# Keyteer/Mixed-precision_LU_Factorization

Hardware: AMD Instinct MI355X
Metric: LU GFLOP/s at N=32768 (1/2/4/8 GPUs); IR iterations to ||r||/||b||<1e-12 (higher is better)
Workload: dtype f64

## Files before the change

### mixed-precision_lu_factorization_amd/csrc/laswp.hip

```cpp
#include "mpf_internal.h"

constexpr int LASWP_CPB = 16;

__global__ __launch_bounds__(256) void laswp_plan_kernel(const int *ipiv, int k, int cols, MovedList *out) {
    __shared__ int slot[HP_MAXCOLS];
    __shared__ int rowof[2 * HP_MAXCOLS];
    __shared__ int content[2 * HP_MAXCOLS];
    __shared__ int used[2 * HP_MAXCOLS];
    __shared__ int count;
    const int t = threadIdx.x;
    for (int s = t; s < 2 * cols; s += 256) { content[s] = s; used[s] = s < cols; rowof[s] = s < cols ? k + s : -1; }
    if (t == 0) count = 0;
    __syncthreads();
    if (t < cols) {
        const int p = ipiv[t] - 1;
        int s;
        if (p < k + cols) s = p - k;
        else {
            int first = t;
            for (int i = 0; i < t; ++i)
                if (ipiv[i] - 1 == p) { first = i; break; }
            s = cols + first;
            if (first == t) { rowof[s] = p; used[s] = 1; }
        }
// ... 308 lines not shown
int launch_cvt_f64_f32(mpf_ctx *c, const double *A, int64_t lda, float *W, int64_t ldw, int64_t rows, int64_t cols) {
    if (rows <= 0 || cols <= 0) return 0;
    if ((cols + 63) / 64 > 65535) { c->err = "cvt: too many columns"; return -1; }
    dim3 grid((unsigned)((rows + 63) / 64), (unsigned)((cols + 63) / 64));
    cvt_a64_wt32_kernel<<<grid, 256, 0, c->stream>>>(A, lda, W, ldw, rows, cols);
    MPF_HIP_TRY(c, hipGetLastError());
    return 0;
}
int launch_cvt_f32_f64(mpf_ctx *c, const float *W, int64_t ldw, double *A, int64_t lda, int64_t rows, int64_t cols) {
    if (rows <= 0 || cols <= 0) return 0;
    if ((cols + 63) / 64 > 65535) { c->err = "cvt: too many columns"; return -1; }
    dim3 grid((unsigned)((rows + 63) / 64), (unsigned)((cols + 63) / 64));
    cvt_wt32_a64_kernel<<<grid, 256, 0, c->stream>>>(W, ldw, A, lda, rows, cols);
    MPF_HIP_TRY(c, hipGetLastError());
    return 0;
}

__global__ void lazy_init_map_kernel(int *F, int *G, long long n) {
    const long long i = (long long)blockIdx.x * 256 + threadIdx.x;
    if (i < n) { F[i] = (int)i; G[i] = (int)i; }
}
__global__ __launch_bounds__(512) void lazy_update_map_kernel(int *F, int *G, const MovedList *ml) {
    int n = ml->n;
    if (n > LASWP_MAXMOVED) n = LASWP_MAXMOVED;
    const int t = threadIdx.x;
    int v = 0;
    if (t < n) v = F[ml->dst[t]];
    __syncthreads();
    if (t < n) { const int s = ml->src[t]; F[s] = v; G[v] = s; }
}
__global__ __launch_bounds__(256) void lazy_gather_kernel(const double *__restrict__ A, long long lda, long long n, long long r0,
                                                         int w, const int *__restrict__ G, double *__restrict__ T, long long ldt) {
    const long long d = r0 + (long long)blockIdx.x * 256 + threadIdx.x;
    if (d >= n) return;
    const long long sr = G[d];
    const int c0 = blockIdx.y * 16;
#pragma unroll 8
    for (int c = c0; c < c0 + 16 && c < w; ++c) T[(d - r0) + (long long)c * ldt] = A[sr + (long long)c * lda];
}
__global__ __launch_bounds__(256) void lazy_scatter_kernel(const double *__restrict__ A, long long lda, long long n, long long r0,
                                                          int w, const int *__restrict__ F, double *__restrict__ T, long long ldt) {
    const long long r = r0 + (long long)blockIdx.x * 256 + threadIdx.x;
    if (r >= n) return;
    const long long d = (long long)F[r] - r0;
    const int c0 = blockIdx.y * 16;
#pragma unroll 4
    for (int c = c0; c < c0 + 16 && c < w; ++c) T[d + (long long)c * ldt] = A[r + (long long)c * lda];
}
__global__ __launch_bounds__(256) void lazy_copyback_kernel(double *__restrict__ A, long long lda, long long n, long long r0, int w,
                                                           const double *__restrict__ T, long long ldt) {
    const long long r = r0 + (long long)blockIdx.x * 256 + threadIdx.x;
    if (r >= n) return;
    const int c0 = blockIdx.y * 16;
#pragma unroll 4
    for (int c = c0; c < c0 + 16 && c < w; ++c) A[r + (long long)c * lda] = T[(r - r0) + (long long)c * ldt];
}

int launch_lazy_left_swaps(mpf_ctx *c, double *A, int64_t lda, int64_t N, int nb, int npanels, const MovedList *lists, int sb,
                           int world, int rank) {
    if (npanels < 2) return 0;
    if (sb < 1 || world > 1) sb = 1;
    const int gather = c->tune.lazy_gather;
    int *Gmap = c->Fmap + N;
    lazy_init_map_kernel<<<(int)((N + 255) / 256), 256, 0, c->stream>>>(c->Fmap, Gmap, N);
    for (int p = npanels - 1; p >= 1; --p) {
        lazy_update_map_kernel<<<1, 512, 0, c->stream>>>(c->Fmap, Gmap, lists + p);
        if (p % sb) continue;
        const int64_t r0 = (int64_t)p * nb;
        const int64_t rows = N - r0;
        if (rows <= 0) continue;
        for (int b = p - sb; b < p; ++b) {
            if (world > 1 && b % world != rank) continue;
            const int w = nb;
            dim3 grid((unsigned)((rows + 255) / 256), (unsigned)((w + 15) / 16));
            double *Ab = A + (int64_t)(world > 1 ? b / world : b) * nb * lda;
            if (gather) lazy_gather_kernel<<<grid, 256, 0, c->stream>>>(Ab, lda, N, r0, w, Gmap, c->perm_tmp, rows);
            else lazy_scatter_kernel<<<grid, 256, 0, c->stream>>>(Ab, lda, N, r0, w, c->Fmap, c->perm_tmp, rows);
            lazy_copyback_kernel<<<grid, 256, 0, c->stream>>>(Ab, lda, N, r0, w, c->perm_tmp, rows);
        }
    }
    MPF_HIP_TRY(c, hipGetLastError());
    return 0;
}
```

### mixed-precision_lu_factorization_amd/csrc/mpf_host.cpp

```cpp
#include "mpf_internal.h"
#include "../../include/MPF.h"
#include <climits>
#include <cstdio>
#include <cstdlib>
#include <cstring>
#include <cmath>
#include <iostream>
#include <vector>
#include <mutex>
#include <functional>
#include <chrono>

static thread_local std::string g_noctx_err;

namespace {
struct OptDesc { const char *name, *env; size_t off; bool wide; long long lo, hi; };
#define OPT_I(field, env, lo, hi) {#field, env, offsetof(MpfTuning, field), false, lo, hi}
#define OPT_L(field, env, lo, hi) {#field, env, offsetof(MpfTuning, field), true, lo, hi}
const OptDesc kOpts[] = {
    OPT_I(safe_pivots, "MPF_SAFE_PIVOTS", 0, 1),
    OPT_I(chain_pipeline, "MPF_CHAIN_PIPELINE", 0, 1),
    OPT_L(chain_pipeline_below, "MPF_CHAIN_PIPELINE_BELOW", 0, 1ll << 40),
    OPT_I(fp16_work32, "MPF_FP16_WORK32", 0, 1),
    OPT_I(superpanel_fp16, "MPF_SUPERPANEL", 0, 8),
    OPT_I(superpanel_fp64, "MPF_SUPERPANEL_FP64", 1, 8),
    OPT_I(no_lookahead, "MPF_NO_LOOKAHEAD", 0, 1),
    OPT_I(verbose, "MPF_VERBOSE", 0, 1),
    OPT_I(timeline, "MPF_TIMELINE", 0, 1),
    OPT_L(hp_spin_limit, "MPF_HP_SPIN_LIMIT", 1, 1ll << 31),
    OPT_L(hp_gate_ticks, "MPF_HP_GATE_TICKS", 0, 1ll << 40),
    OPT_I(hp_acq_fence, "MPF_HP_ACQ_FENCE", 0, 1),
    OPT_I(hp_window, "MPF_HP_WINDOW", -1, 1 << 30),
    OPT_I(hgemm_pad, "MPF_HGEMM_PAD", 0, 65536),
    OPT_I(hgemm_split_pad, "MPF_HGEMM_SPLIT_PAD", 0, 65536),
    OPT_I(hgemm_big, "MPF_HGEMM_BIG", 0, 1),
    OPT_I(hgemm_big_tile, "MPF_HGEMM_BIG_TILE", 0, 5),
    OPT_I(hgemm_mfma16, "MPF_HGEMM_MFMA16", 0, 1),
    OPT_I(dgemm_dma, "MPF_DGEMM_DMA", 0, 1),
    OPT_I(lazy_gather, "MPF_LAZY_GATHER", 0, 1),
    OPT_I(dpanel_fused_form, "MPF_DPANEL_FUSED", 0, 1),
    OPT_I(dist_instalments, "MPF_DIST_INSTALMENTS", 0, 1),
    OPT_L(dist_instalment_min_bytes, "MPF_DIST_INSTALMENT_MIN_BYTES", 0, 1ll << 40),
    OPT_I(generic_fused, "MPF_GENERIC_FUSED", 0, 1),
    OPT_I(fp64_rowmajor, "MPF_FP64_ROWMAJOR", 0, 1),
    OPT_L(fp64_rowmajor_min_n, "MPF_FP64_ROWMAJOR_MIN_N", 0, 1ll << 40),
    OPT_I(trsm_laswp_fused, "MPF_TRSM_LASWP_FUSED", 0, 1),
    OPT_I(fp64_two_lanes, "MPF_FP64_TWO_LANES", 0, 1 << 30),
    OPT_I(fp64_lane_a_pct, "MPF_FP64_LANE_A_PCT", 20, 90),
    OPT_I(event_timers, "MPF_EVENT_TIMERS", 0, 2),
    OPT_I(dist_world1_loop, "MPF_DIST_WORLD1_LOOP", 0, 1),
    OPT_I(gesv_fp64_tflops, "MPF_GESV_FP64_TFLOPS", 0, 1000),
    OPT_I(gate_wait_value, "MPF_GATE_WAIT_VALUE", 0, 1),
    OPT_I(host_sink, "MPF_HOST_SINK", 0, 1),
    OPT_I(sink_trace, "MPF_SINK_TRACE", 0, 1),
    OPT_I(hp_half_slabs, "MPF_HP_HALF_SLABS", 0, 1),
    OPT_I(hp_half_slabs_rows, "MPF_HP_HALF_SLABS_ROWS", 256, 32768),
    OPT_I(hp_local_xcd, "MPF_HP_LOCAL_XCD", 0, 2),
    OPT_I(host_late_parts, "MPF_HOST_LATE_PARTS", 0, 4),
    OPT_L(host_late_min_n, "MPF_HOST_LATE_MIN_N", 0, 1ll << 40),
    OPT_I(host_first_pct, "MPF_HOST_FIRST_PCT", 5, 100),
    OPT_I(host_late_q_pct, "MPF_HOST_LATE_Q_PCT", 1, 1000),
    OPT_L(host_sink_min_n, "MPF_HOST_SINK_MIN_N", 0, 1ll << 40),
    OPT_I(dist_solve_p2p, "MPF_DIST_SOLVE_P2P", 0, 1),
#ifdef MPF_PROBE
    OPT_I(hp_stamp, "MPF_HP_STAMP", 0, 1),
    OPT_I(hp_r256_upto, "MPF_HP_R256_UPTO", 0, 1 << 30),
    OPT_I(dgemm_w8, "MPF_DGEMM_W8", 0, 1),
    OPT_I(gemm_lds_pad, "MPF_GEMM_LDS_PAD", 0, 65536),
    OPT_I(hgemm_big_reg, "MPF_HGEMM_BIG_REG", 0, 1),
    OPT_I(hgemm_dbg, "MPF_HGEMM_DBG", 0, 8191),
#endif
};
#undef OPT_I
#undef OPT_L
void opt_store(MpfTuning &t, const OptDesc &d, long long v) {
    if (v < d.lo) v = d.lo;
    if (v > d.hi) v = d.hi;
    char *p = (char *)&t + d.off;
    if (d.wide) *(long long *)p = v; else *(int *)p = (int)v;
}
long long opt_load(const MpfTuning &t, const OptDesc &d) {
    const char *p = (const char *)&t + d.off;
    return d.wide ? *(const long long *)p : (long long)*(const int *)p;
}
void tuning_from_env(MpfTuning &t) {
    for (const OptDesc &d : kOpts)
        if (const char *e = getenv(d.env)) if (*e) opt_store(t, d, atoll(e));
}
}

static int fail(mpf_ctx *c, int code, const std::string &msg) {
    if (c) c->err = msg; else g_noctx_err = msg;
    return code;
}

extern "C" {

int mpf_create(mpf_ctx **out, int device) {
    if (!out) return -1;
    *out = nullptr;
    int ndev = 0;
    hipError_t e = hipGetDeviceCount(&ndev);
    if (e != hipSuccess || ndev == 0) return fail(nullptr, -3, "No HIP devices available.");
    if (device < 0 || device >= ndev) return fail(nullptr, -1, "mpf_create: bad device index");
    mpf_ctx *c = new mpf_ctx();
    tuning_from_env(c->tune);
    c->device = device;
    if (hipSetDevice(device) != hipSuccess) { delete c; return fail(nullptr, -2, "hipSetDevice failed"); }
    hipDeviceProp_t prop;
    if (hipGetDeviceProperties(&prop, device) == hipSuccess) c->num_cus = prop.multiProcessorCount;
    if (hipStreamCreateWithFlags(&c->stream, hipStreamNonBlocking) != hipSuccess) { delete c; return fail(nullptr, -2, "hipStreamCreate failed"); }
    c->own_stream = true;
    {
        int lo = 0, hi = 0;
        hipDeviceGetStreamPriorityRange(&lo, &hi);
        if (hipStreamCreateWithPriority(&c->pstream, hipStreamNonBlocking, hi) != hipSuccess) c->pstream = nullptr;
        if (hipStreamCreateWithPriority(&c->tstream, hipStreamNonBlocking, hi) != hipSuccess) c->tstream = nullptr;
    }
    if (hipMalloc((void **)&c->ws, sizeof(MpfWorkspace)) != hipSuccess) { hipStreamDestroy(c->stream); delete c; return fail(nullptr, -2, "hipMalloc(workspace) failed"); }
    hipMemset(c->ws, 0, sizeof(MpfWorkspace));
    if (hipExtMallocWithFlags((void **)&c->hp_signal, 8, hipMallocSignalMemory) != hipSuccess) { c->hp_signal = nullptr; (void)hipGetLastError(); }
    else hipMemset(c->hp_signal, 0, 8);
// ... 437 lines not shown
        const int64_t ns = has_next ? pc2 : n;
        rc = ev.timed(st.ms_trsm, S, [&] { return launch_dtrsm_llnu(c, pc, ns, Ap, lda, A12, lda); });
        if (rc) break;
        rc = ev.timed(st.ms_gemm, S, [&] {
            int e = o.trailing != MPF_TRAIL_FP64 ? launch_cvt_l21(c, Ap + pc, lda, n, pc, o.trailing == MPF_TRAIL_FP16X3) : 0;
            if (!e) e = trail_gemm(c, o, n, ns, pc, Ap + pc, A12, A12 + pc, lda);
            return e; });
        if (rc) break;
        count_gemm(st, o, n, ns, pc);
        if (!has_next) break;
        hipEvent_t e1 = ev.get(), e2 = ev.get();
        hipEventRecord(e1, S);
        hipEvent_t e2p = nullptr, e2t = nullptr;
        int rcp = 0;
        const bool piped = chain_pipelined(c, ev, st, o, d_A, lda, N, nx, pc2, d_ipiv, c->lists + (nx / nb), e1, &e2p, &e2t, &rcp) == 0;
        if (piped) rc = rcp;
        else {
            hipStreamWaitEvent(P, e1, 0);
            StreamSwap sw(c, P);
            double *Anx = d_A + nx * lda + nx;
            MovedList *ml = c->lists + (nx / nb);
            rc = ev.timed(st.ms_hpanel, P, [&] {
                return launch_hgetf2(c, Anx, lda, nullptr, 0, (int)(N - nx), pc2, (int)nx, d_ipiv + nx, nullptr, 0, ml, 0, o.trailing == MPF_TRAIL_FP64 ? HP_FP64_WINDOW_ROWS : 0); });
            if (!rc) rc = ev.timed(st.ms_dpanel, P, [&] {
                int e = launch_laswp_from_list(c, d_A + nx * lda, lda, pc2, ml);
                if (!e) e = launch_dgetf2_npv(c, Anx, lda, (int)(N - nx), pc2, o.fused_panel, (int)nx);
                return e;
            });
        }
        if (rc) break;
        if (!piped) hipEventRecord(e2, P);
        st.panels++;
        if (n > pc2) {
            rc = ev.timed(st.ms_laswp, S, [&] {
                return launch_laswp_from_list(c, d_A + (nx + pc2) * lda, lda, N - nx - pc2, c->lists + (k / nb)); });
            if (rc) break;
            double *A12r = A12 + (int64_t)pc2 * lda;
            rc = ev.timed(st.ms_trsm, S, [&] { return launch_dtrsm_llnu(c, pc, n - pc2, Ap, lda, A12r, lda); });
            if (rc) break;
            if (sink) sink_notify(c, (int)(k / nb) + 1, S);
            rc = ev.timed(st.ms_gemm, S, [&] { return trail_gemm(c, o, n, n - pc2, pc, Ap + pc, A12r, A12r + pc, lda); });
            if (rc) break;
            count_gemm(st, o, n, n - pc2, pc);
        }
        if (piped) { hipStreamWaitEvent(S, e2p, 0); hipStreamWaitEvent(S, e2t, 0); }
        else hipStreamWaitEvent(S, e2, 0);
        rc = ev.timed(st.ms_laswp, S, [&] {
            const int64_t s0 = nx + pc2;
            const int64_t sw = (N - s0) < nb ? (N - s0) : nb;
            return sw > 0 ? launch_laswp_from_list(c, d_A + s0 * lda, lda, sw, c->lists + (nx / nb)) : 0;
        });
        if (o.verbose) printf("panel k=%lld rows=%lld cols=%d (look-ahead)\n", (long long)nx, (long long)(N - nx), pc2);
    }
    if (sink) {
        hipEvent_t ep = ev.get(); hipEventRecord(ep, P); hipStreamWaitEvent(S, ep, 0);
        sink_notify(c, (int)((N + nb - 1) / nb), S);
    } else if (!rc) rc = ev.timed(st.ms_laswp, S, [&] { return launch_lazy_left_swaps(c, d_A, lda, N, nb, (int)((N + nb - 1) / nb), c->lists); });
    hipError_t se = sink_stream_wait(c, S);
    hipError_t sp = sink_stream_wait(c, P);
    if (c->tstream) { const hipError_t stt = sink_stream_wait(c, c->tstream); if (sp == hipSuccess) sp = stt; }
    if (!rc && (se != hipSuccess || sp != hipSuccess))
        return fail(c, -2, std::string("factorization failed: ") + hipGetErrorString(se != hipSuccess ? se : sp));
    ev.collect();
    st.lookahead = 1;
    return rc;
}

static int factor_lookahead_rm(mpf_ctx *c, double *d_A, int64_t lda, int64_t N, int32_t nb, int32_t *d_ipiv,
                               const mpf_opts &o, mpf_stats &st) {
    hipStream_t S = c->stream, P = c->pstream, T = c->tstream;
    EvPool ev(c);
    ev.keep = &st.ms_gemm;
    int rc = 0;
    const bool sink = sink_take(c, d_A, lda, N, nb);
    double *R = c->r64;
    const int64_t ldr = N;
    LatePlan *lp = (c->late && !c->late->taken && c->late->nseg > 0 && lda == N) ? c->late : nullptr;
    if (lp) lp->taken = true;
    int lseg = 0;
    int64_t ce = lp ? lp->c0[0] : N;
    { hipEvent_t e = ev.get(); hipEventRecord(e, S); hipStreamWaitEvent(P, e, 0); if (T) hipStreamWaitEvent(T, e, 0); }
    const int pc0 = (int)(N < nb ? N : nb);
    hipEvent_t chain_a = nullptr, chain_b = nullptr;
    if (N > 1) {
        hipEvent_t e0 = ev.get();
        {
            StreamSwap sw(c, P);
            rc = ev.timed(st.ms_hpanel, P, [&] {
                int e = launch_hgetf2(c, d_A, lda, nullptr, 0, (int)N, pc0, 0, d_ipiv, nullptr, 0, c->lists, 0, o.trailing == MPF_TRAIL_FP64 ? HP_FP64_WINDOW_ROWS : 0);
                if (!e) e = launch_laswp_from_list(c, d_A, lda, pc0, c->lists);
                if (!e) e = launch_dgetf2_npv(c, d_A, lda, (int)N, pc0, o.fused_panel, 0);
                return e; });
            hipEventRecord(e0, P);
        }
        st.panels++;
        if (!rc && pc0 < ce) rc = ev.timed(st.ms_cvt, S, [&] { return launch_transpose64(c, d_A + (int64_t)pc0 * lda, lda, R + pc0, ldr, N, ce - pc0, true); });
        hipStreamWaitEvent(S, e0, 0);
        chain_a = e0;
    }
    int64_t cm = -1;
    hipEvent_t doneL = nullptr, doneR = nullptr, prevR = nullptr;
    hipEvent_t init_done = ev.get();
    hipEventRecord(init_done, S);
    bool was_two = false;
    for (int64_t k = 0; k < N && rc == 0; k += nb) {
        const int pc = (int)((N - k) < nb ? (N - k) : nb);
        if (N - k <= 1 || k + pc >= N) break;
        const int64_t n = N - k - pc;
        const int64_t nx = k + pc;
        const int pc2 = (int)((N - nx) < nb ? (N - nx) : nb);
        const bool has_next = (N - nx) > 1;
        double *Ap = d_A + k * lda + k;
        double *LT = c->rm_lt + ((k / nb) & 1) * N * (int64_t)nb;
        const int64_t ns = has_next ? pc2 : n;
        MovedList *lk = c->lists + (k / nb);
        while (lp && lseg < lp->nseg && (k / nb >= lp->q[lseg] || nx + pc2 > ce || !has_next)) {
            const int64_t c_lo = lp->c0[lseg], c_hi = lseg + 1 < lp->nseg ? lp->c0[lseg + 1] : N, w = c_hi - c_lo;
            double *LT3 = c->rm_lt + 2 * N * (int64_t)nb;
            rc = launch_late_wait(c, lp->flags + lseg, lp->seq);
            if (!rc && lp->snapshot) {
                MPF_HIP_TRY(c, hipMemcpyAsync(lp->snapshot + c_lo * N, d_A + c_lo * lda, (size_t)w * N * sizeof(double), hipMemcpyDeviceToDevice, S));
                lp->snapped[lseg] = true;
            }
            if (!rc) rc = ev.timed(st.ms_cvt, S, [&] { return launch_transpose64(c, d_A + c_lo * lda, lda, R + c_lo, ldr, N, w, true); });
            for (int64_t kj = 0; kj < k && rc == 0; kj += nb) {
                const int64_t nxj = kj + nb, nj = N - nxj;
                double *Apj = d_A + kj * lda + kj;
                const MovedList *lj = c->lists + (kj / nb);
                rc = ev.timed(st.ms_cvt, S, [&] { return launch_transpose64(c, Apj + nb, lda, LT3, nb, nj, nb, true); });
                if (!rc) rc = ev.timed(st.ms_laswp, S, [&] { return launch_laswp_from_list_rm64(c, R + c_lo, ldr, w, lj, (int64_t)LASWP_MAXMOVED * c_lo); });
                if (!rc) rc = ev.timed(st.ms_trsm, S, [&] { return launch_dtrsm_llnu_strided(c, nb, w, Apj, lda, R + kj * ldr + c_lo, ldr, 1); });
                if (!rc) rc = ev.timed(st.ms_cvt, S, [&] { return launch_transpose64(c, d_A + c_lo * lda + kj, lda, R + kj * ldr + c_lo, ldr, nb, w, false); });
                if (!rc) rc = ev.timed(st.ms_gemm, S, [&] { return launch_dgemm_minus(c, w, nj, nb, R + kj * ldr + c_lo, ldr, LT3, nb, R + nxj * ldr + c_lo, ldr); });
                count_gemm(st, o, nj, w, nb);
                if (sink && !rc && c_hi == N) sink_notify(c, (int)(kj / nb) + 1, S);
            }
            ++lseg;
            ce = lseg < lp->nseg ? lp->c0[lseg] : N;
            cm = -1;
            doneR = ev.get();
            hipEventRecord(doneR, S);
            doneL = nullptr;
        }
        if (rc) break;
        const int64_t cw = ce - nx - pc2;
        const bool pivots_fit = c->num_cus <= 0 || (N - nx + HP_R - 1) / HP_R <= (int64_t)c->num_cus * 4 / 5;
        const bool want_two = T && c->tune.fp64_two_lanes > 0 && has_next && pivots_fit && (N - nx) > c->tune.chain_pipeline_below &&
                              cw >= c->tune.fp64_two_lanes;
        bool resplit = false;
        if (!want_two) cm = -1;
        else if (cm < 0 || (cm - (nx + pc2)) * 100 < cw * (c->tune.fp64_lane_a_pct - 10)) {
            cm = nx + pc2 + ((cw * c->tune.fp64_lane_a_pct / 100 + 127) / 128) * 128;
            if (cm > ce - 128) cm = ce - 128;
            resplit = true;
        }
        if (cm >= 0) {
            const int64_t aw = cm - (nx + pc2);
            if (!was_two && k > 0) {
                doneL = ev.get();
                hipEventRecord(doneL, S);
            }
            hipEvent_t lt_ready = ev.get();
            {
                if (prevR) hipStreamWaitEvent(P, prevR, 0);
                StreamSwap sw(c, P);
                rc = ev.timed(st.ms_cvt, P, [&] { return launch_transpose64(c, Ap + pc, lda, LT, pc, n, pc, true); });
// ... 57 lines not shown
            if (rc) break;
            count_gemm(st, o, n, ce - cm, pc);
            prevR = doneR;
            doneR = ev.get();
            hipEventRecord(doneR, S);
            chain_a = e2; chain_b = nullptr;
            was_two = true;
            if (o.verbose) printf("panel k=%lld rows=%lld cols=%d (look-ahead, row-major copy, two lanes split at %lld)\n", (long long)nx, (long long)(N - nx), pc2, (long long)cm);
            continue;
        }
        if (was_two) {
            hipEvent_t et = ev.get(); hipEventRecord(et, T); hipStreamWaitEvent(S, et, 0);
            if (chain_a) hipStreamWaitEvent(S, chain_a, 0);
            if (chain_b) hipStreamWaitEvent(S, chain_b, 0);
            was_two = false;
        }
        hipEvent_t lt_ready = ev.get();
        {
            hipEvent_t eb = ev.get();
            hipEventRecord(eb, S);
            hipStreamWaitEvent(P, eb, 0);
            StreamSwap sw(c, P);
            rc = ev.timed(st.ms_cvt, P, [&] { return launch_transpose64(c, Ap + pc, lda, LT, pc, n, pc, true); });
            hipEventRecord(lt_ready, P);
        }
        if (!rc) rc = ev.timed(st.ms_laswp, S, [&] { return launch_laswp_from_list_rm64(c, R + nx, ldr, ce - nx, lk); });
        if (!rc) rc = ev.timed(st.ms_trsm, S, [&] { return launch_dtrsm_llnu_strided(c, pc, ns, Ap, lda, R + k * ldr + nx, ldr, 1); });
        hipStreamWaitEvent(S, lt_ready, 0);
        if (!rc) rc = ev.timed(st.ms_gemm, S, [&] { return launch_dgemm_minus(c, ns, n, pc, R + k * ldr + nx, ldr, LT, pc, R + nx * ldr + nx, ldr); });
        if (rc) break;
        count_gemm(st, o, n, ns, pc);
        if (!has_next) {
            rc = ev.timed(st.ms_cvt, S, [&] {
                int e = launch_transpose64(c, d_A + nx * lda + k, lda, R + k * ldr + nx, ldr, pc, N - nx, false);
                if (!e) e = launch_transpose64(c, d_A + nx * lda + nx, lda, R + nx * ldr + nx, ldr, N - nx, N - nx, false);
                return e; });
            break;
        }
        rc = ev.timed(st.ms_cvt, S, [&] { return launch_transpose64(c, d_A + nx * lda + nx, lda, R + nx * ldr + nx, ldr, N - nx, pc2, false); });
        if (rc) break;
        hipEvent_t e1 = ev.get(), e2 = ev.get();
        hipEventRecord(e1, S);
        hipEvent_t e2p = nullptr, e2t = nullptr;
        int rcp = 0;
        const bool piped = chain_pipelined(c, ev, st, o, d_A, lda, N, nx, pc2, d_ipiv, c->lists + (nx / nb), e1, &e2p, &e2t, &rcp) == 0;
        if (piped) rc = rcp;
        else {
            hipStreamWaitEvent(P, e1, 0);
            StreamSwap sw(c, P);
            double *Anx = d_A + nx * lda + nx;
            MovedList *ml = c->lists + (nx / nb);
            rc = ev.timed(st.ms_hpanel, P, [&] {
                return launch_hgetf2(c, Anx, lda, nullptr, 0, (int)(N - nx), pc2, (int)nx, d_ipiv + nx, nullptr, 0, ml, 0, o.trailing == MPF_TRAIL_FP64 ? HP_FP64_WINDOW_ROWS : 0); });
            if (!rc) rc = ev.timed(st.ms_dpanel, P, [&] {
                int e = launch_laswp_from_list(c, d_A + nx * lda, lda, pc2, ml);
                if (!e) e = launch_dgetf2_npv(c, Anx, lda, (int)(N - nx), pc2, o.fused_panel, (int)nx);
                return e;
            });
        }
        if (rc) break;
        if (!piped) hipEventRecord(e2, P);
        st.panels++;
        if (cw > 0) {
            rc = ev.timed(st.ms_trsm, S, [&] { return launch_dtrsm_llnu_strided(c, pc, cw, Ap, lda, R + k * ldr + nx + pc2, ldr, 1); });
            if (rc) break;
        }
        if (T) {
            hipEvent_t eu = ev.get();
            hipEventRecord(eu, S);
            hipStreamWaitEvent(T, eu, 0);
            StreamSwap sw(c, T);
            rc = ev.timed(st.ms_cvt, T, [&] { return launch_transpose64(c, d_A + nx * lda + k, lda, R + k * ldr + nx, ldr, pc, ce - nx, false); });
            if (sink && !rc && ce == N) sink_notify(c, (int)(k / nb) + 1, T);
        } else {
            rc = ev.timed(st.ms_cvt, S, [&] { return launch_transpose64(c, d_A + nx * lda + k, lda, R + k * ldr + nx, ldr, pc, ce - nx, false); });
            if (sink && !rc && ce == N) sink_notify(c, (int)(k / nb) + 1, S);
        }
        if (rc) break;
        if (cw > 0) {
            rc = ev.timed(st.ms_gemm, S, [&] { return launch_dgemm_minus(c, cw, n, pc, R + k * ldr + nx + pc2, ldr, LT, pc, R + nx * ldr + nx + pc2, ldr); });
            if (rc) break;
            count_gemm(st, o, n, cw, pc);
        }
        if (piped) { hipStreamWaitEvent(S, e2p, 0); hipStreamWaitEvent(S, e2t, 0); chain_a = e2p; chain_b = e2t; }
        else { hipStreamWaitEvent(S, e2, 0); chain_a = e2; chain_b = nullptr; }
        if (o.verbose) printf("panel k=%lld rows=%lld cols=%d (look-ahead, row-major copy)\n", (long long)nx, (long long)(N - nx), pc2);
    }
    if (!rc && lp && lseg < lp->nseg) rc = fail(c, -1, "factor_lookahead_rm: a late column segment was never brought up to date (plan beyond the matrix)");
    if (T) { hipEvent_t et = ev.get(); hipEventRecord(et, T); hipStreamWaitEvent(S, et, 0); }
    { hipEvent_t ep = ev.get(); hipEventRecord(ep, P); hipStreamWaitEvent(S, ep, 0); }
    if (sink) sink_notify(c, (int)((N + nb - 1) / nb), S);
    else if (!rc) rc = ev.timed(st.ms_laswp, S, [&] { return launch_lazy_left_swaps(c, d_A, lda, N, nb, (int)((N + nb - 1) / nb), c->lists); });
    hipError_t se = sink_stream_wait(c, S);
    hipError_t sp = sink_stream_wait(c, P);
    if (T) { const hipError_t stt = sink_stream_wait(c, T); if (sp == hipSuccess) sp = stt; }
    if (!rc && (se != hipSuccess || sp != hipSuccess))
        return fail(c, -2, std::string("factorization failed: ") + hipGetErrorString(se != hipSuccess ? se : sp));
    ev.collect();
    st.lookahead = 1;
    return rc;
}

static int factor_superpanel(mpf_ctx *c, double *d_A, int64_t lda, int64_t N, int32_t nb, int32_t *d_ipiv, const mpf_opts &o,
                             mpf_stats &st, int sb, bool overlap) {
    hipStream_t S = c->stream, P = overlap ? c->pstream : c->stream;
    hipStream_t Ci = (overlap && c->tstream) ? c->tstream : c->stream;
    const bool lanes = Ci != S;
    EvPool ev(c);
    ev.keep = &st.ms_gemm;
    int rc = 0;
    const bool split = o.trailing == MPF_TRAIL_FP16X3;
    const bool f64 = o.trailing == MPF_TRAIL_FP64;
    const bool use32 = !f64 && c->tune.fp16_work32 != 0 && N > (int64_t)(sb + 1) * nb;
    float *W = nullptr;
    const int64_t ldw = N;
    if (use32) {
        if (c->w32_n < N) {
            if (c->w32) (void)hipFree(c->w32);
            c->w32 = nullptr; c->w32_n = 0;
            MPF_HIP_TRY(c, hipMalloc((void **)&c->w32, (size_t)N * (size_t)N * sizeof(float)));
            c->w32_n = N;
        }
        W = c->w32;
    }
    if (overlap) {
        hipEvent_t e = ev.get();
        hipEventRecord(e, S);
        hipStreamWaitEvent(P, e, 0);
    }
    const int64_t sbw = (int64_t)sb * nb;
    const int kst = (int)((sbw + 63) & ~(int64_t)63);
    const int64_t far_cap = N - (int64_t)(sb + 1) * nb;
    const int64_t inner_u_off = (!f64 && far_cap > 0) ? far_cap * kst : 0;
    const int64_t brow_l_off = (int64_t)N * c->h_kmax;
    auto width = [&](int64_t k) { return (int)((N - k) < nb ? (N - k) : nb); };
    auto chain = [&](int64_t kx, hipStream_t s) -> int {
        const int pcx = width(kx);
        const int prx = (int)(N - kx);
        if (prx <= 1) return 0;
        StreamSwap sw(c, s);
        double *Ax = d_A + kx * lda + kx;
        MovedList *ml = c->lists + (kx / nb);
        int e = ev.timed(st.ms_hpanel, s, [&] { return launch_hgetf2(c, Ax, lda, nullptr, 0, prx, pcx, (int)kx, d_ipiv + kx, nullptr, 0, ml, 0, o.trailing == MPF_TRAIL_FP64 ? HP_FP64_WINDOW_ROWS : 0); });
        if (!e) e = ev.timed(st.ms_dpanel, s, [&] {
            int e2 = launch_laswp_from_list(c, d_A + kx * lda, lda, pcx, ml);
            if (!e2) e2 = launch_dgetf2_npv(c, Ax, lda, prx, pcx, o.fused_panel, (int)kx);
            return e2; });
        st.panels++;
        return e;
    };
    auto side_chain = [&](int64_t kx, hipEvent_t e1, hipEvent_t &e2) -> int {
        if (!overlap) return chain(kx, S);
        e2 = ev.get();
        if (N - kx > 1) {
            hipEvent_t e2p = nullptr, e2t = nullptr;
            int rcp = 0;
            if (chain_pipelined(c, ev, st, o, d_A, lda, N, kx, width(kx), d_ipiv, c->lists + (kx / nb), e1, &e2p, &e2t, &rcp) == 0) {
                st.panels++;
                if (!rcp) { hipStreamWaitEvent(c->tstream, e2p, 0); hipEventRecord(e2, c->tstream); }
                return rcp;
            }
        }
        hipStreamWaitEvent(P, e1, 0);
        int e = chain(kx, P);
        hipEventRecord(e2, P);
        return e;
    };
    hipEvent_t img_ready = nullptr;
    auto l21_image = [&](int64_t k, int pc) -> int {
        if (f64) return 0;
        const int64_t mrows = N - k - pc;
        if (mrows <= 0) return 0;
        hipStream_t Is = (lanes && P != S) ? P : Ci;
        if (Is != Ci) { hipEvent_t e = ev.get(); hipEventRecord(e, Ci); hipStreamWaitEvent(Is, e, 0); }
        StreamSwap sw(c, Is);
// ... 555 lines not shown
```

### mixed-precision_lu_factorization_amd/csrc/mpf_internal.h

```cpp
#pragma once
#include <hip/hip_runtime.h>
#include <stdint.h>
#include <string>
#include <vector>
#include <functional>
#include "../../include/mpf_c.h"

constexpr int HP_R = 256;
constexpr int HP_T = 512;
constexpr int HP_MAXG = 256;
constexpr int HP_MAXCOLS = 256;
constexpr int LASWP_MAXMOVED = 2 * HP_MAXCOLS;

struct MovedList {
    int n;
    int pad[3];
    int src[LASWP_MAXMOVED];
    int dst[LASWP_MAXMOVED];
};

struct MpfWorkspace {
    unsigned long long cand[2][HP_MAXG];
    int flags[16];
    unsigned long long rowbuf[2][HP_MAXG][HP_MAXCOLS / 2];
    int hp_timeouts;
    int pad0[3];
    MovedList list0;
    int info;
    int pad[3];
    unsigned long long hp_stamps[8];
    unsigned long long hp_progress;
    unsigned long long hp_xcd_target;
    unsigned long long hp_xcd_roles;
};

struct MpfTuning {
    int safe_pivots = 0;
    int chain_pipeline = 1;
    long long chain_pipeline_below = 10240;
    int fp16_work32 = 1;
    int superpanel_fp16 = 0;
    int superpanel_fp64 = 1;
    int no_lookahead = 0;
    int verbose = 0;
    int timeline = 0;
    long long hp_spin_limit = 1ll << 21;
    long long hp_gate_ticks = 200000000ll;
    int hp_window = -1;
    int hp_acq_fence = 0;
    int hgemm_pad = 0;
    int hgemm_split_pad = 32768;
    int hgemm_big = 1;
    int hgemm_mfma16 = 1;
    int hgemm_big_tile = 0;
    int dgemm_dma = 1;
    int lazy_gather = 1;
    int dpanel_fused_form = 1;
    int dist_instalments = 1;
    long long dist_instalment_min_bytes = 8ll << 20;
    int generic_fused = 1;
    int fp64_rowmajor = 1;
    long long fp64_rowmajor_min_n = 8192;
    int trsm_laswp_fused = 1;
    int fp64_two_lanes = 8192;
    int dist_solve_p2p = 0;
    int host_sink = 1;
    int hp_local_xcd = 1;
    int hp_half_slabs = 1;
    int hp_half_slabs_rows = 16384;
    int sink_trace = 0;
    int host_late_parts = 3;
    long long host_late_min_n = 16384;
    int host_first_pct = 25;
    int host_late_q_pct = 110;
    long long host_sink_min_n = 4096;
    int gate_wait_value = 0;
    int gesv_fp64_tflops = 0;
    int dist_world1_loop = 0;
    int event_timers = 1;
    int fp64_lane_a_pct = 50;
#ifdef MPF_PROBE
    int hp_stamp = 0;
    int hp_r256_upto = 1 << 30;
    int dgemm_w8 = 1;
    int gemm_lds_pad = 0;
    int hgemm_dbg = 0;
    int hgemm_big_reg = 0;
#endif
};

struct mpf_ctx {
    MpfTuning tune;
    unsigned attr_done = 0;
    unsigned attr_big = 0;
    int device = 0;
    hipStream_t stream = nullptr;
    bool own_stream = false;
    hipStream_t pstream = nullptr;
    hipStream_t tstream = nullptr;
    hipStream_t xstream = nullptr;
    std::vector<hipEvent_t> ev_pool;
    MpfWorkspace *ws = nullptr;
    hipEvent_t ev0 = nullptr, ev1 = nullptr;
    std::string err;
    mpf_stats stats{};
    int num_cus = 0;
    double *solve_buf = nullptr;
    int64_t solve_n = 0;
    unsigned short *h_L = nullptr, *h_U = nullptr;
    int64_t h_rows = 0;
    unsigned short *h_Lb[2] = {nullptr, nullptr};
    int h_kmax = 0;
    unsigned hp_seq = 0;
    unsigned long long *hp_signal = nullptr;
    int32_t *perm_buf = nullptr;
    MovedList *lists = nullptr;
    int lists_cap = 0;
    int *Fmap = nullptr;
    double *perm_tmp = nullptr;
    int64_t perm_cap = 0, fmap_cap = 0;
    double *trsv_inv = nullptr;
    double *trsv_inv256 = nullptr;
    int *trsv_cnt = nullptr;
    double *krylov = nullptr;
    size_t krylov_cap = 0;
    double *res_part = nullptr;
    size_t res_part_cap = 0;
    double *dtiles = nullptr;
    int dtiles_cap = 0;
    float *w32 = nullptr;
    int64_t w32_n = 0;
    double *r64 = nullptr;
    int64_t r64_n = 0;
    int64_t r64_cap = 0;
    bool hgemm_standalone = false;
    mpf_p2p_fn p2p_fn = nullptr;
    void *p2p_user = nullptr;
    double gmres_budget_ms = 0;
    double fp64_rate_tflops = 0;
    double *host_A = nullptr;
    int64_t host_A_cap = 0;
    int32_t *host_P = nullptr;
    int64_t host_P_cap = 0;
    double *host_A0 = nullptr;
    int64_t host_A0_cap = 0;
    unsigned *late_flags = nullptr;
    unsigned late_seq = 0;
    struct ColFeed *feed = nullptr;
    struct LatePlan *late = nullptr;
    struct RowSink *sink = nullptr;
    double *rm_tmp = nullptr;
    int64_t rm_tmp_cap = 0;
    double *rm_lt = nullptr;
    int64_t rm_lt_cap = 0;
    unsigned short *g16 = nullptr;
    size_t g16_cap = 0;
    unsigned long long *gcand = nullptr;
    int gcand_cap = 0;
    void *rccl_comm = nullptr;
    int rccl_rank = 0, rccl_world = 0;
    long long rccl_bcast_calls = 0, rccl_bcast_bytes = 0, rccl_allreduce_calls = 0, rccl_p2p_calls = 0, rccl_p2p_bytes = 0;
    double *dist_buf[2] = {nullptr, nullptr};
    size_t dist_buf_cap = 0;
    float *dist_w32 = nullptr;
    int64_t dist_w32_cap = 0;
    double *dist_spl = nullptr;
    int64_t dist_spl_cap = 0;
    int hp_resident_per_cu = -1;
    int hp_win_per_cu = 0;
    int hp_full_beside_waiter = 0;
    int hp_win_beside_waiter = 0;
};

#define MPF_HIP_TRY(ctx, expr)                                                        \
    do {                                                                              \
        hipError_t e_ = (expr);                                                       \
        if (e_ != hipSuccess) {                                                       \
            (ctx)->err = std::string(#expr) + ": " + hipGetErrorString(e_);           \
            return -2;                                                                \
        }                                                                             \
    } while (0)

enum { ATTR_HP = 1, ATTR_DGEMM = 2, ATTR_HGEMM = 4, ATTR_HGEMM256 = 8, ATTR_HGEMM_PP = 16, ATTR_HGEMM16_BIG32 = 32, ATTR_HGEMM16_BIG64 = 64 };
inline bool safe_pivots(const mpf_ctx *c) { return c->tune.safe_pivots != 0; }

int launch_double_to_fp16(mpf_ctx *c, const double *in, uint16_t *out, int64_t n);
int launch_hdiv(mpf_ctx *c, const uint16_t *a, const uint16_t *b, uint16_t *q, int64_t n);
int launch_hgetf2(mpf_ctx *c, const double *A64, int64_t lda, uint16_t *P16, int64_t ld16, int rows,
                  int cols, int ipiv_offset, int *d_ipiv, uint16_t *out16, int64_t ldo, MovedList *moved, int waiters = 0, int prefer_window_rows = 0);
bool hgetf2_lds_eligible(mpf_ctx *c, int rows, int cols);
bool hgetf2_fits_beside(mpf_ctx *c, int rows, int cols, int waiters);
long long hgetf2_capacity_rows(mpf_ctx *c, int waiters, int form = 0);
int laswp_gated_footprint(int *lds_bytes, int *vgprs, int *threads);
int laswp_gated_grid(int64_t ncols);
constexpr int HP_FP64_WINDOW_ROWS = 20000;
int hp_query_residency(mpf_ctx *c);
int launch_hgetf2_gate(mpf_ctx *c, int target);
int launch_laswp_block(mpf_ctx *c, double *A, int64_t lda, int64_t ncols, int k, int cols, const int *d_ipiv, int64_t nrows);
int launch_laswp_block_gated(mpf_ctx *c, double *A, int64_t lda, int64_t ncols, int k, int cols, const int *d_ipiv, int64_t nrows, int target);
int dgetf2_npv_pieces(mpf_ctx *c, int cols);
int launch_dgetf2_npv_piece(mpf_ctx *c, double *P, int64_t ld, int rows, int cols, int fused, int info_base, int piece);
int launch_dpanel_tile_copy(mpf_ctx *c, double *dst, int64_t ld, int piece);
int launch_hgetf2_generic(mpf_ctx *c, const double *A64, int64_t lda, uint16_t *P16, int64_t ld16, int rows, int cols,
                          int ipiv_offset, int *d_ipiv, uint16_t *out16, int64_t ldo);
int launch_laswp_seq(mpf_ctx *c, double *A, int64_t lda, int64_t ncols, int k, int cols, const int *d_ipiv, int64_t nrows);
int launch_laswp_from_list(mpf_ctx *c, double *A, int64_t lda, int64_t ncols, const MovedList *ml);
int launch_laswp_from_list_hole(mpf_ctx *c, double *A, int64_t lda, int64_t ncols, const MovedList *ml, int64_t hole_from, int64_t hole_len);
int launch_lazy_left_swaps(mpf_ctx *c, double *A, int64_t lda, int64_t N, int nb, int npanels, const MovedList *lists, int sb = 1,
                           int world = 1, int rank = 0);
struct LatePlan {
    int nseg = 0;
    int64_t c0[4] = {0, 0, 0, 0};
    int q[4] = {0, 0, 0, 0};
    unsigned *flags = nullptr;
    unsigned seq = 0;
    double *snapshot = nullptr;
    bool taken = false;
    bool snapped[4] = {false, false, false, false};
};
int launch_late_wait(mpf_ctx *c, const unsigned *flag, unsigned seq);
int feed_start(mpf_ctx *c, const double *A_host, double *d_A, int64_t N, LatePlan *lp);
int feed_finish(mpf_ctx *c);
void feed_destroy(mpf_ctx *c);
void feed_trim(mpf_ctx *c);
int sink_attach(mpf_ctx *c, double *A_host, int64_t N, int nb);
bool sink_take(mpf_ctx *c, const double *d_A, int64_t lda, int64_t N, int nb);
void sink_notify(mpf_ctx *c, int upto_panel, hipStream_t stream);
hipError_t sink_stream_wait(mpf_ctx *c, hipStream_t stream);
int sink_finish(mpf_ctx *c, int *panels_sent);
void sink_destroy(mpf_ctx *c);
void sink_trim(mpf_ctx *c);
int launch_laswp(mpf_ctx *c, double *A, int64_t lda, int64_t ncols, int k, int cols, const int *d_ipiv);
int launch_laswp_plan(mpf_ctx *c, const int *d_ipiv, int k, int cols, MovedList *out);
int launch_dgetf2_npv(mpf_ctx *c, double *P, int64_t ld, int rows, int cols, int fused, int info_base);
int launch_dtrsm_llnu(mpf_ctx *c, int m, int64_t n, const double *L, int64_t ldl, double *B, int64_t ldb);
int launch_dgemm_minus(mpf_ctx *c, int64_t m, int64_t n, int k, const double *A, int64_t lda,
                       const double *B, int64_t ldb, double *C, int64_t ldc);
int launch_cvt_l21(mpf_ctx *c, const double *A, int64_t lda, int64_t m, int K, int split, int img = 0, int64_t elem_off = 0);
int launch_hgemm_minus(mpf_ctx *c, int64_t m, int64_t n, int K, const double *B, int64_t ldb, double *C, int64_t ldc,
                       int split, int img = 0, int64_t elem_off = 0);
int launch_hgemm_minus_w32(mpf_ctx *c, int64_t m, int64_t n, int K, const double *B, int64_t ldb, float *C, int64_t ldc,
                           int split, int img = 0, int64_t elem_off = 0);
int launch_cvt_u12(mpf_ctx *c, const double *B, int64_t ldb, int K, int64_t n, int split, int64_t elem_off = 0, int kstride = 0);
int launch_hgemm_images(mpf_ctx *c, int64_t m, int64_t n, int K, void *C, int64_t ldc, bool c32, int split, int img = 0, int64_t elem_off = 0,
                        int64_t u_off = 0, int ksL = 0, int ksU = 0);
struct HgemmImages { const unsigned short *Lh = nullptr, *Ll = nullptr, *Uh = nullptr, *Ul = nullptr; int ksL = 0, ksU = 0; };
int launch_hgemm_ptrs(mpf_ctx *c, int64_t m, int64_t n, int K, const HgemmImages &im, void *C, int64_t ldc, bool c32, int split);
int launch_hgemm16_big(mpf_ctx *c, int64_t m, int64_t n, int Kp, const HgemmImages &im, void *C, int64_t ldc, bool c32);
int launch_hgemm16_ring(mpf_ctx *c, int64_t m, int64_t n, int Kp, const HgemmImages &im, void *C, int64_t ldc, bool c32);
int launch_hgemm_pp(mpf_ctx *c, int64_t m, int64_t n, int Kp, const HgemmImages &im, float *C, int64_t ldc);
int launch_hgemm_images_rowmajor(mpf_ctx *c, int64_t m, int64_t n, int K, float *Crm, int64_t ldrow, int split, int img = 0, int64_t elem_off = 0,
                                 int64_t u_off = 0, int ksL = 0, int ksU = 0);
int launch_laswp_from_list_f32(mpf_ctx *c, float *A, int64_t lda, int64_t ncols, const MovedList *ml);
int launch_laswp_from_list_rm64(mpf_ctx *c, double *R, int64_t ldr, int64_t ncols, const MovedList *ml, int64_t scratch_off = 0);
int launch_transpose64(mpf_ctx *c, double *A, int64_t lda, double *R, int64_t ldr, int64_t rows, int64_t cols, bool to_rowmajor);
int launch_dtrsm_llnu_strided(mpf_ctx *c, int m, int64_t n, const double *L, int64_t ldl, double *B, int64_t rs, int64_t cs);
int launch_cvt_f64_f32(mpf_ctx *c, const double *A, int64_t lda, float *W, int64_t ldw, int64_t rows, int64_t cols);
int launch_cvt_f32_f64(mpf_ctx *c, const float *W, int64_t ldw, double *A, int64_t lda, int64_t rows, int64_t cols);
int launch_gather_rows(mpf_ctx *c, const double *in, const int *perm, double *out, int64_t n);
int launch_residual(mpf_ctx *c, const double *A, int64_t lda, const double *x, const double *b, double *r,
                    int64_t n);
int launch_residual_rect(mpf_ctx *c, const double *A, int64_t lda, const double *x, const double *b, double *r, int64_t n, int64_t ncols);
int launch_trsv_prepare_cols(mpf_ctx *c, const double *LUb, int64_t ld, int64_t n, int64_t k0, int w);
int launch_trsv_lower_cols(mpf_ctx *c, const double *LUb, int64_t ld, double *x, int64_t n, int64_t k0, int w);
int launch_trsv_upper_cols(mpf_ctx *c, const double *LUb, int64_t ld, double *x, int64_t n, int64_t k0, int w);
extern "C" {
int mpf_ensure_h_images(mpf_ctx *c, int64_t rows, int kmax, bool big);
int mpf_ensure_solve_buf(mpf_ctx *c, int64_t n);
int mpf_ensure_rowmajor_copy(mpf_ctx *c, int64_t rows, int64_t cols, int32_t nb);
}
int launch_trsv_prepare(mpf_ctx *c, const double *LU, int64_t ld, int64_t n);
int launch_trsv_lower_unit(mpf_ctx *c, const double *LU, int64_t ld, double *x, int64_t n);
int launch_trsv_upper(mpf_ctx *c, const double *LU, int64_t ld, double *x, int64_t n);
int launch_axpy(mpf_ctx *c, double alpha, const double *x, double *y, int64_t n);
int launch_norm2(mpf_ctx *c, const double *x, int64_t n, double *d_out);
int launch_dot(mpf_ctx *c, const double *x, const double *y, int64_t n, double *d_out);
int launch_scal(mpf_ctx *c, double alpha, double *x, int64_t n);

struct StreamSwap {
    mpf_ctx *c; hipStream_t saved;
    StreamSwap(mpf_ctx *c_, hipStream_t s) : c(c_), saved(c_->stream) { c->stream = s; }
    ~StreamSwap() { c->stream = saved; }
};
struct EvPool {
    mpf_ctx *c; size_t next = 0;
    struct Pair { hipEvent_t a, b; double *acc, *acc2; };
    std::vector<Pair> pairs;
    const double *keep = nullptr;
    explicit EvPool(mpf_ctx *c_) : c(c_) {}
    hipEvent_t get() {
        if (next == c->ev_pool.size()) { hipEvent_t e; hipEventCreate(&e); c->ev_pool.push_back(e); }
        return c->ev_pool[next++];
// ... 35 lines not shown
```

Measured before the change: 53520.

## Split lazy left-swaps: interleave early panels into factorization, batch late panels wide

Adds a lazy_split mode that applies the deferred left-side row swaps in two parts. Panels below a split point are walked in small batches during the look-ahead loop, where they can overlap with other work. The remaining tail is applied at the end with one wide gather/copyback per panel, using the row-major scratch as a temporary. New tiled gather/copyback kernels use an XCD-strided tile assignment. The costs are extra kernel launches inside the main loop and a dependence on the scratch buffers having enough capacity.

```diff
diff --git a/mixed-precision_lu_factorization_amd/csrc/laswp.hip b/mixed-precision_lu_factorization_amd/csrc/laswp.hip
--- a/mixed-precision_lu_factorization_amd/csrc/laswp.hip
+++ b/mixed-precision_lu_factorization_amd/csrc/laswp.hip
@@ -414,3 +414,60 @@
     MPF_HIP_TRY(c, hipGetLastError());
     return 0;
 }
+
+struct LazyTiles {
+    long long X, x, W, nrt, n_u;
+    __device__ LazyTiles(long long rows, long long w) {
+        X = (gridDim.x >= 8 && (gridDim.x & 7) == 0) ? 8 : 1;
+        x = blockIdx.x % X; W = gridDim.x / X;
+        nrt = (rows + 255) / 256;
+        const long long nst = (w + 15) / 16;
+        n_u = ((nst - x + X - 1) / X) * nrt;
+    }
+    __device__ long long first() const { return blockIdx.x / X; }
+    __device__ long long row(long long u) const { return (u % nrt) * 256; }
+    __device__ long long col(long long u) const { return (x + X * (u / nrt)) * 16; }
+};
+__global__ __launch_bounds__(256) void lazy_gather_tiles_kernel(const double *__restrict__ A, long long lda, long long n, long long r0,
+                                                               long long w, const int *__restrict__ G, double *__restrict__ T, long long ldt) {
+    const LazyTiles lt(n - r0, w);
+    for (long long u = lt.first(); u < lt.n_u; u += lt.W) {
+        const long long d = r0 + lt.row(u) + threadIdx.x, c0 = lt.col(u);
+        if (d >= n) continue;
+        const long long sr = G[d];
+#pragma unroll 8
+        for (long long c = c0; c < c0 + 16 && c < w; ++c) T[(d - r0) + c * ldt] = A[sr + c * lda];
+    }
+}
+__global__ __launch_bounds__(256) void lazy_copyback_tiles_kernel(double *__restrict__ A, long long lda, long long n, long long r0, long long w,
+                                                                 const double *__restrict__ T, long long ldt) {
+    const LazyTiles lt(n - r0, w);
+    for (long long u = lt.first(); u < lt.n_u; u += lt.W) {
+        const long long r = r0 + lt.row(u) + threadIdx.x, c0 = lt.col(u);
+        if (r >= n) continue;
+#pragma unroll 4
+        for (long long c = c0; c < c0 + 16 && c < w; ++c) A[r + c * lda] = T[(r - r0) + c * ldt];
+    }
+}
+int launch_lazy_left_walk(mpf_ctx *c, double *A, int64_t lda, int64_t N, int nb, int p_top, int p_bot, const MovedList *lists, bool wide,
+                          double *T, int64_t tcap, bool init_map) {
+    if (p_bot < 1 || p_top < p_bot) return 0;
+    if ((int64_t)p_top * nb >= N) { c->err = "lazy left walk: panel beyond the matrix"; return -1; }
+    const int64_t r_bot = (int64_t)p_bot * nb;
+    if ((N - r_bot) * (wide ? r_bot : (int64_t)nb) > tcap) { c->err = "lazy left walk: scratch too small"; return -1; }
+    int *Gmap = c->Fmap + N;
+    if (init_map) lazy_init_map_kernel<<<(int)((N + 255) / 256), 256, 0, c->stream>>>(c->Fmap, Gmap, N);
+    for (int p = p_top; p >= p_bot; --p) {
+        lazy_update_map_kernel<<<1, 512, 0, c->stream>>>(c->Fmap, Gmap, lists + p);
+        const int64_t r0 = (int64_t)p * nb, rows = N - r0;
+        const int64_t w = (wide && p == p_bot) ? r0 : nb;
+        double *Ab = A + (r0 - w) * lda;
+        long long tiles = ((rows + 255) / 256) * ((w + 15) / 16);
+        long long grid = (tiles + 7) / 8 * 8;
+        if (grid > (1ll << 30)) grid = 1ll << 30;
+        lazy_gather_tiles_kernel<<<(unsigned)grid, 256, 0, c->stream>>>(Ab, lda, N, r0, w, Gmap, T, rows);
+        lazy_copyback_tiles_kernel<<<(unsigned)grid, 256, 0, c->stream>>>(Ab, lda, N, r0, w, T, rows);
+    }
+    MPF_HIP_TRY(c, hipGetLastError());
+    return 0;
+}
diff --git a/mixed-precision_lu_factorization_amd/csrc/mpf_host.cpp b/mixed-precision_lu_factorization_amd/csrc/mpf_host.cpp
--- a/mixed-precision_lu_factorization_amd/csrc/mpf_host.cpp
+++ b/mixed-precision_lu_factorization_amd/csrc/mpf_host.cpp
@@ -38,6 +38,7 @@
     OPT_I(hgemm_mfma16, "MPF_HGEMM_MFMA16", 0, 1),
     OPT_I(dgemm_dma, "MPF_DGEMM_DMA", 0, 1),
     OPT_I(lazy_gather, "MPF_LAZY_GATHER", 0, 1),
+    OPT_I(lazy_split, "MPF_LAZY_SPLIT", 0, 1),
     OPT_I(dpanel_fused_form, "MPF_DPANEL_FUSED", 0, 1),
     OPT_I(dist_instalments, "MPF_DIST_INSTALMENTS", 0, 1),
     OPT_L(dist_instalment_min_bytes, "MPF_DIST_INSTALMENT_MIN_BYTES", 0, 1ll << 40),
@@ -641,6 +642,16 @@
     { hipEvent_t e = ev.get(); hipEventRecord(e, S); hipStreamWaitEvent(P, e, 0); if (T) hipStreamWaitEvent(T, e, 0); }
     const int pc0 = (int)(N < nb ? N : nb);
     hipEvent_t chain_a = nullptr, chain_b = nullptr;
+    const int npanels = (int)((N + nb - 1) / nb);
+    int q_split = -1;
+    if (c->tune.lazy_split && !sink && !lp && c->perm_tmp && c->Fmap) {
+        const int64_t cpb = c->tune.chain_pipeline_below;
+        int64_t q = N - cpb <= 0 ? 1 : (N - cpb + nb - 1) / nb;
+        if (q < 1) q = 1;
+        if (q <= npanels - 2) q_split = (int)q;
+    }
+    int early_next = q_split;
+    const int early_per = q_split > 0 ? (q_split + (npanels - 3 - q_split)) / (npanels - 2 - q_split > 0 ? npanels - 2 - q_split : 1) : 0;
     if (N > 1) {
         hipEvent_t e0 = ev.get();
         {
@@ -864,6 +875,12 @@
             if (rc) break;
             count_gemm(st, o, n, cw, pc);
         }
+        if (q_split > 0 && nx > (int64_t)q_split * nb && early_next >= 1) {
+            const int p_bot = early_next - early_per + 1 > 1 ? early_next - early_per + 1 : 1;
+            rc = ev.timed(st.ms_laswp, S, [&] { return launch_lazy_left_walk(c, d_A, lda, N, nb, early_next, p_bot, c->lists, false, c->perm_tmp, c->perm_cap, early_next == q_split); });
+            early_next = p_bot - 1;
+            if (rc) break;
+        }
         if (piped) { hipStreamWaitEvent(S, e2p, 0); hipStreamWaitEvent(S, e2t, 0); chain_a = e2p; chain_b = e2t; }
         else { hipStreamWaitEvent(S, e2, 0); chain_a = e2; chain_b = nullptr; }
         if (o.verbose) printf("panel k=%lld rows=%lld cols=%d (look-ahead, row-major copy)\n", (long long)nx, (long long)(N - nx), pc2);
@@ -872,7 +889,12 @@
     if (T) { hipEvent_t et = ev.get(); hipEventRecord(et, T); hipStreamWaitEvent(S, et, 0); }
     { hipEvent_t ep = ev.get(); hipEventRecord(ep, P); hipStreamWaitEvent(S, ep, 0); }
     if (sink) sink_notify(c, (int)((N + nb - 1) / nb), S);
-    else if (!rc) rc = ev.timed(st.ms_laswp, S, [&] { return launch_lazy_left_swaps(c, d_A, lda, N, nb, (int)((N + nb - 1) / nb), c->lists); });
+    else if (!rc && q_split > 0)
+        rc = ev.timed(st.ms_laswp, S, [&] {
+            int e = launch_lazy_left_walk(c, d_A, lda, N, nb, early_next, 1, c->lists, false, c->perm_tmp, c->perm_cap, early_next == q_split);
+            if (!e) e = launch_lazy_left_walk(c, d_A, lda, N, nb, npanels - 1, q_split + 1, c->lists, true, R, c->r64_cap, true);
+            return e; });
+    else if (!rc) rc = ev.timed(st.ms_laswp, S, [&] { return launch_lazy_left_swaps(c, d_A, lda, N, nb, npanels, c->lists); });
     hipError_t se = sink_stream_wait(c, S);
     hipError_t sp = sink_stream_wait(c, P);
     if (T) { const hipError_t stt = sink_stream_wait(c, T); if (sp == hipSuccess) sp = stt; }
diff --git a/mixed-precision_lu_factorization_amd/csrc/mpf_internal.h b/mixed-precision_lu_factorization_amd/csrc/mpf_internal.h
--- a/mixed-precision_lu_factorization_amd/csrc/mpf_internal.h
+++ b/mixed-precision_lu_factorization_amd/csrc/mpf_internal.h
@@ -55,6 +55,7 @@
     int hgemm_big_tile = 0;
     int dgemm_dma = 1;
     int lazy_gather = 1;
+    int lazy_split = 1;
     int dpanel_fused_form = 1;
     int dist_instalments = 1;
     long long dist_instalment_min_bytes = 8ll << 20;
@@ -208,6 +209,8 @@
 int launch_laswp_from_list_hole(mpf_ctx *c, double *A, int64_t lda, int64_t ncols, const MovedList *ml, int64_t hole_from, int64_t hole_len);
 int launch_lazy_left_swaps(mpf_ctx *c, double *A, int64_t lda, int64_t N, int nb, int npanels, const MovedList *lists, int sb = 1,
                            int world = 1, int rank = 0);
+int launch_lazy_left_walk(mpf_ctx *c, double *A, int64_t lda, int64_t N, int nb, int p_top, int p_bot, const MovedList *lists, bool wide,
+                          double *T, int64_t tcap, bool init_map);
 struct LatePlan {
     int nseg = 0;
     int64_t c0[4] = {0, 0, 0, 0};
```

After: 53730 (median of 6 runs). About the same (+0.4%).
